# jdubkim/Self-play-on-Multi-Snakes-Environment

Measured on AMD Instinct MI355X. Metric: env-steps/sec (agent·step) at 4 096×19×19×3-snake, 1/2/4/8 GPU + CPU ref, higher is better.
Workload: dtype u8

## Files before the change

### include/msnake.h

```cpp
#ifndef MSNAKE_H
#define MSNAKE_H

#include <stddef.h>
#include <stdint.h>

#ifdef __cplusplus
extern "C" {
#endif

#define MSNAKE_ABI_VERSION 3

#define MSNAKE_RULES_SNAKE_ENV 0
#define MSNAKE_RULES_NEW_WORLD 1
#define MSNAKE_RULES_ADVERSARIAL 2

#define MSNAKE_MAX_SNAKES 4
#define MSNAKE_MAX_FRUITS 32
#define MSNAKE_MAX_DIM 62

#define MSNAKE_OK 0
#define MSNAKE_E_ARG (-1)
#define MSNAKE_E_HIP (-2)
#define MSNAKE_E_HANDLE (-3)
#define MSNAKE_E_ALIGN (-4)
// ... 81 lines not shown
int msnake_state_blob_info(const void* buf, size_t bytes, msnake_blob_info* out);

int msnake_render(msnake_handle h, uint8_t* obs_dev, void* stream);

#define MSNAKE_POLICY_NONE 0
#define MSNAKE_POLICY_SAFE_GREEDY 1
#define MSNAKE_POLICY_HAMILTONIAN 2
int msnake_scripted_actions(msnake_handle h, int32_t policy, uint32_t snake_mask, int32_t* actions_dev,
                            int32_t action_stride, uint8_t* safe_dev, void* stream);

int msnake_copy_envs(msnake_handle dst, msnake_handle src, const int32_t* src_index_dev, void* stream);

int msnake_get_stats(msnake_handle h, msnake_stats* out, int32_t reset);

const char* msnake_kernel_name(msnake_handle h);
int64_t msnake_algorithmic_bytes_per_env_step(msnake_handle h);

#ifdef __cplusplus
}
#endif
#endif
```

### self-play-on-multi-snakes-environment_amd/_capi.py

```python
import ctypes
import os

_HERE = os.path.dirname(os.path.abspath(__file__))
LIB_PATH = os.environ.get("MSNAKE_LIB") or os.path.join(_HERE, "libmsnake.so")

RULES = {"snake_env": 0, "new_world": 1, "adversarial": 2}
RULE_NAMES = {v: k for k, v in RULES.items()}

SYMBOLS = [
    "msnake_abi_version", "msnake_last_error", "msnake_create", "msnake_destroy", "msnake_obs_shape",
    "msnake_reset", "msnake_reset_envs", "msnake_step", "msnake_step_tape", "msnake_rollout_tape", "msnake_get_state", "msnake_set_state",
    "msnake_get_state_all", "msnake_set_state_all", "msnake_state_blob_info",
    "msnake_render", "msnake_get_stats", "msnake_kernel_name", "msnake_algorithmic_bytes_per_env_step",
    "msnake_scripted_actions", "msnake_copy_envs",
]


class MsnakeConfig(ctypes.Structure):
    _fields_ = [("struct_size", ctypes.c_uint32), ("device", ctypes.c_int32), ("num_envs", ctypes.c_int32),
                ("dim", ctypes.c_int32), ("n_snakes", ctypes.c_int32), ("n_fruits", ctypes.c_int32),
                ("rules", ctypes.c_int32), ("max_steps", ctypes.c_int32), ("auto_reset", ctypes.c_int32),
                ("obs_scale", ctypes.c_int32), ("seed", ctypes.c_uint64), ("env_id_base", ctypes.c_uint64),
                ("envs_per_block", ctypes.c_int32), ("record_policy", ctypes.c_int32),
                ("obs_store_policy", ctypes.c_int32), ("tape_store_policy", ctypes.c_int32)]


ABI_VERSION = 3
CONFIG_SIZE_V2 = 56
RECORD_POLICY = {"auto": 0, "full": 1, "short": 2}
# ... 39 lines not shown
    L.msnake_reset_envs.argtypes = [vp, u8p, u8p, u8p, u8p, vp]
    L.msnake_step.argtypes = [vp, vp, i32, u8p, vp, vp, vp, vp]
    L.msnake_scripted_actions.argtypes = [vp, i32, ctypes.c_uint32, vp, i32, u8p, vp]
    L.msnake_copy_envs.argtypes = [vp, vp, vp, vp]
    L.msnake_step_tape.argtypes = [vp, vp, i32, i32, u8p, ctypes.c_size_t, vp, vp, vp, ctypes.c_size_t, vp]
    L.msnake_rollout_tape.argtypes = L.msnake_step_tape.argtypes
    L.msnake_get_state.argtypes = [vp, i32, vp, i32]
    L.msnake_set_state.argtypes = [vp, i32, vp, i32]
    L.msnake_get_state_all.argtypes = [vp, vp, ctypes.c_size_t]
    L.msnake_get_state_all.restype = ctypes.c_int64
    L.msnake_set_state_all.argtypes = [vp, vp, ctypes.c_size_t]
    L.msnake_state_blob_info.argtypes = [vp, ctypes.c_size_t, ctypes.POINTER(MsnakeBlobInfo)]
    L.msnake_get_stats.argtypes = [vp, ctypes.POINTER(MsnakeStats), i32]
    L.msnake_kernel_name.argtypes = [vp]
    L.msnake_kernel_name.restype = ctypes.c_char_p
    L.msnake_algorithmic_bytes_per_env_step.argtypes = [vp]
    L.msnake_algorithmic_bytes_per_env_step.restype = ctypes.c_int64
    for name in ("msnake_create", "msnake_destroy", "msnake_obs_shape", "msnake_reset", "msnake_reset_envs", "msnake_render",
                 "msnake_step", "msnake_step_tape", "msnake_rollout_tape", "msnake_get_state", "msnake_set_state", "msnake_set_state_all",
                 "msnake_state_blob_info", "msnake_get_stats", "msnake_scripted_actions", "msnake_copy_envs"):
        getattr(L, name).restype = ctypes.c_int
    _lib = L
    return L


def check(rc, what="msnake call"):
    if rc < 0:
        msg = load().msnake_last_error().decode("utf-8", "replace")
        raise RuntimeError(f"{what} failed ({rc}): {msg}")
    return rc
```

### self-play-on-multi-snakes-environment_amd/csrc/msnake_capi.hip

```cpp
#include <hip/hip_runtime.h>

#include <cstdarg>
#include <cstdio>
#include <cstdlib>
#include <cstring>
#include <vector>

#include "msnake_internal.h"

namespace {

thread_local char g_err[512] = "";

int fail(int code, const char* fmt, ...) {
    va_list ap;
    va_start(ap, fmt);
    vsnprintf(g_err, sizeof(g_err), fmt, ap);
    va_end(ap);
    return code;
}

#define HIP_TRY(expr)                                                                                   \
    do {                                                                                                \
        hipError_t _e = (expr);                                                                         \
// ... 55 lines not shown
        case 2: return "snake count differs from the handle's";
        case 3: return "fruit count differs from the handle's (or exceeds the fruit-list capacity)";
        case 4: return "a cell lies outside [-1, dim], or a body piece behind the head outside the grid";
        case 5: return "a body length is outside [0, capacity]";
        default: return "malformed state";
    }
}

}

extern "C" {

int msnake_abi_version(void) { return MSNAKE_ABI_VERSION; }
const char* msnake_last_error(void) { return g_err; }

int msnake_create(const msnake_config* cfg_in, msnake_handle* out) {
    if (!cfg_in || !out) return fail(MSNAKE_E_ARG, "msnake_create: NULL argument");
    *out = nullptr;
    if (cfg_in->struct_size != sizeof(msnake_config) && cfg_in->struct_size != MSNAKE_CONFIG_SIZE_V2)
        return fail(MSNAKE_E_ARG, "msnake_config.struct_size %u is neither %zu (ABI 3) nor %u (ABI 2)", cfg_in->struct_size,
                    sizeof(msnake_config), MSNAKE_CONFIG_SIZE_V2);
    msnake_config cfg_full;
    memset(&cfg_full, 0, sizeof(cfg_full));
    memcpy(&cfg_full, cfg_in, cfg_in->struct_size);
    cfg_full.struct_size = (uint32_t)sizeof(msnake_config);
    const msnake_config* cfg = &cfg_full;
    if (cfg->num_envs < 1) return fail(MSNAKE_E_ARG, "num_envs must be >= 1 (got %d)", cfg->num_envs);
    if (cfg->dim < 2 || cfg->dim > MSNAKE_MAX_DIM)
        return fail(MSNAKE_E_ARG, "dim must be in [2, %d] (got %d)", MSNAKE_MAX_DIM, cfg->dim);
    if (cfg->rules != MSNAKE_RULES_SNAKE_ENV && cfg->rules != MSNAKE_RULES_NEW_WORLD &&
        cfg->rules != MSNAKE_RULES_ADVERSARIAL)
        return fail(MSNAKE_E_ARG, "rules %d is not one of MSNAKE_RULES_*", cfg->rules);
    if (cfg->rules == MSNAKE_RULES_NEW_WORLD) {
        if (cfg->n_snakes < 1 || cfg->n_snakes > MSNAKE_MAX_SNAKES)
            return fail(MSNAKE_E_ARG, "new_world: n_snakes must be in [1, %d]", MSNAKE_MAX_SNAKES);
        if (cfg->n_fruits < 0 || cfg->n_fruits > MSNAKE_MAX_FRUITS)
            return fail(MSNAKE_E_ARG, "new_world: n_fruits must be in [0, %d]", MSNAKE_MAX_FRUITS);
    } else {
        if (cfg->n_snakes < 1 || cfg->n_snakes > 3)
            return fail(MSNAKE_E_ARG, "snake_env: n_snakes must be in [1, 3] (got %d)", cfg->n_snakes);
        if (cfg->n_fruits != cfg->n_snakes)
// ... 1 lines not shown
    }
    if (cfg->max_steps < 1 || cfg->max_steps > 60000)
        return fail(MSNAKE_E_ARG, "max_steps must be in [1, 60000]");
    if ((uint64_t)cfg->num_envs * (uint64_t)(MSNAKE_HDR_WORDS * 4 + MSNAKE_MAX_SNAKES * 128) >= (1ull << 32))
        return fail(MSNAKE_E_ARG, "num_envs %d: records and body rings of one handle must stay below 4 GB (the kernel "
                                  "addresses them with 32-bit offsets); use several handles", cfg->num_envs);
    if (cfg->obs_scale != 1 && cfg->obs_scale != 4 && cfg->obs_scale != 7)
        return fail(MSNAKE_E_ARG, "obs_scale must be 1, 4 (21->84) or 7 (12->84), got %d", cfg->obs_scale);
    if (cfg->envs_per_block < 0 || cfg->envs_per_block > MSNAKE_MAX_ENVS_PER_BLOCK)
        return fail(MSNAKE_E_ARG, "envs_per_block must be 0 (auto) or in [1, %d], got %d", MSNAKE_MAX_ENVS_PER_BLOCK, cfg->envs_per_block);
    if (cfg->record_policy < 0 || cfg->record_policy > MSNAKE_RECORD_SHORT)
        return fail(MSNAKE_E_ARG, "record_policy must be MSNAKE_AUTO, MSNAKE_RECORD_FULL or MSNAKE_RECORD_SHORT, got %d", cfg->record_policy);
    if (cfg->obs_store_policy < 0 || cfg->obs_store_policy > MSNAKE_STORE_STREAM || cfg->tape_store_policy < 0 ||
        cfg->tape_store_policy > MSNAKE_STORE_STREAM)
        return fail(MSNAKE_E_ARG, "obs_store_policy / tape_store_policy must be MSNAKE_AUTO, MSNAKE_STORE_PLAIN or MSNAKE_STORE_STREAM");

    int ndev = 0;
    if (hipGetDeviceCount(&ndev) != hipSuccess || ndev < 1)
        return fail(MSNAKE_E_NOGPU, "no HIP device available (this library has no CPU path)");
    if (cfg->device < 0 || cfg->device >= ndev)
        return fail(MSNAKE_E_ARG, "device %d out of range (have %d)", cfg->device, ndev);
    DeviceGuard guard(cfg->device);

    msnake_env* h = static_cast<msnake_env*>(calloc(1, sizeof(msnake_env)));
    if (!h) return fail(MSNAKE_E_ARG, "out of host memory");
    h->cfg = *cfg;
    msnake::StepParams& p = h->p;
    const int dim = cfg->dim, W = dim + 2, n2 = dim * dim;
    p.nenv = cfg->num_envs;
    p.dim = dim;
    p.n_snakes = cfg->n_snakes;
    p.n_fruits = cfg->n_fruits;
    p.views = cfg->rules == MSNAKE_RULES_NEW_WORLD ? cfg->n_snakes : 3;
    p.C = 3 * p.views;
    p.S = W * W * p.C;
    p.obs_scale = cfg->obs_scale;
    p.rest.max_steps = cfg->max_steps;
    p.auto_reset = cfg->auto_reset ? 1 : 0;
    int need = n2 + 2;
    if (cfg->rules == MSNAKE_RULES_NEW_WORLD && cfg->max_steps + 2 > need) need = cfg->max_steps + 2;
    p.rest.cap = (need + 63) / 64 * 64;
    const int K = cfg->obs_scale;
    if (K > 1 && (W * K * p.C) % 4 != 0) {
        free(h);
        return fail(MSNAKE_E_ARG, "obs_scale %d: output rows must be whole dwords", K);
    }
    p.img_bytes = (p.S * K + (K == 1 ? 15 : 0) + 1023) / 1024 * 1024;
    p.rest.seed_lo = (uint32_t)cfg->seed;
    p.rest.seed_hi = (uint32_t)(cfg->seed >> 32);
    p.rest.env_id_base = cfg->env_id_base;
    p.lds_per_wave = p.img_bytes + (n2 + 15) / 16 * 16;
    h->epb = p.nenv <= 8192 ? MSNAKE_MAX_ENVS_PER_BLOCK : 4;
    while (h->epb > 1 && (size_t)h->epb * p.lds_per_wave > 64 * 1024) h->epb >>= 1;
    if ((size_t)p.lds_per_wave > 64 * 1024 - 16 || p.S > 0xFFFF) {
        free(h);
        return fail(MSNAKE_E_ARG, "observation image of %d bytes does not fit in LDS", p.S);
    }

    const size_t hdr_bytes = (size_t)p.nenv * MSNAKE_HDR_WORDS * 4;
    const size_t body0_bytes = (size_t)p.nenv * p.n_snakes * 64 * 2;
    const int tmpl_copies = K == 1 ? MSNAKE_TMPL_COPIES : 1;
    const size_t tmpl_bytes = (size_t)p.img_bytes * tmpl_copies;
    const size_t ring_bytes = (size_t)p.nenv * p.n_snakes * p.rest.cap * 2;
    const bool adv = cfg->rules == MSNAKE_RULES_ADVERSARIAL;
    p.fcap = (p.n_snakes + p.n_snakes * (n2 + 2) + 63) / 64 * 64;
    const size_t fl0_bytes = adv ? (size_t)p.nenv * 64 * 2 : 0;
    const size_t flist_bytes = adv ? (size_t)p.nenv * p.fcap * 2 : 0;
    const size_t state_bytes = hdr_bytes + body0_bytes + tmpl_bytes + ring_bytes + fl0_bytes + flist_bytes;
    hipError_t e;
    if ((e = hipMalloc(&h->d_state, state_bytes)) != hipSuccess || (e = hipMalloc(&h->d_stats, 64)) != hipSuccess ||
        (e = hipMemset(h->d_state, 0, state_bytes)) != hipSuccess || (e = hipMemset(h->d_stats, 0, 64)) != hipSuccess) {
        (void)hipFree(h->d_state); (void)hipFree(h->d_stats);
// ... 8 lines not shown
    p.fl0 = reinterpret_cast<uint16_t*>(p.state + hdr_bytes + body0_bytes + tmpl_bytes + ring_bytes);
    p.flist = reinterpret_cast<uint16_t*>(p.state + hdr_bytes + body0_bytes + tmpl_bytes + ring_bytes + fl0_bytes);
    p.stats = static_cast<unsigned long long*>(h->d_stats);
    std::vector<uint8_t> tmpl(tmpl_bytes, 0);
    for (int copy = 0; copy < tmpl_copies; ++copy)
        for (int r = 0; r < W; ++r)
            for (int c = 0; c < W; ++c)
                if (r == 0 || r == W - 1 || c == 0 || c == W - 1)
                    memset(&tmpl[(size_t)copy * p.img_bytes + copy + ((size_t)r * W + c) * p.C * K], 255, (size_t)p.C * K);
    if ((e = hipMemcpy(const_cast<uint8_t*>(p.tmpl), tmpl.data(), tmpl_bytes, hipMemcpyHostToDevice)) != hipSuccess) {
        (void)hipFree(h->d_state); (void)hipFree(h->d_stats);
        free(h);
        return fail(MSNAKE_E_HIP, "uploading the background image failed: %s", hipGetErrorString(e));
    }
    if (cfg->envs_per_block > 0 && cfg->envs_per_block < h->epb) h->epb = cfg->envs_per_block;
    p.short_rec = (cfg->rules != MSNAKE_RULES_NEW_WORLD && p.nenv > 8192) ? 1 : 0;
    if (cfg->record_policy != MSNAKE_AUTO)
        p.short_rec = (cfg->rules != MSNAKE_RULES_NEW_WORLD && cfg->record_policy == MSNAKE_RECORD_SHORT) ? 1 : 0;
    {
        const double obs_mib = (double)p.nenv * p.S * p.obs_scale * p.obs_scale / (1024.0 * 1024.0);
        p.rest.stream_obs = (p.obs_scale == 1 ? (obs_mib <= 32.0 || obs_mib >= 192.0) : obs_mib >= 400.0) ? 1u : 0u;
    }
    if (cfg->obs_store_policy != MSNAKE_AUTO) p.rest.stream_obs = cfg->obs_store_policy == MSNAKE_STORE_STREAM ? 1u : 0u;
#ifdef MSNAKE_DBG_STAGES
    if (const char* dbg = getenv("MSNAKE_DBG_STAGE")) p.rest.dbg_stage = (uint32_t)atoi(dbg);
    if (const char* dbg = getenv("MSNAKE_DBG_BUF")) p.rest.dbg_buf = reinterpret_cast<unsigned long long*>(strtoull(dbg, nullptr, 0));
#endif
#if defined(MSNAKE_DBG_STAGES) || defined(MSNAKE_SPAN_LIGHT)
    if (const char* dbg = getenv("MSNAKE_DBG_SPAN")) {
        h->dbg_span = reinterpret_cast<unsigned long long*>(strtoull(dbg, nullptr, 0));
        const char* sl = getenv("MSNAKE_DBG_SPAN_SLOTS");
        h->dbg_span_slots = sl ? (uint32_t)atoi(sl) : 1u;
        if (h->dbg_span_slots < 1) h->dbg_span_slots = 1;
    }
#endif
    msnake::step_kernel_name(cfg->rules, cfg->n_snakes, cfg->obs_scale, h->kname, sizeof(h->kname));
    h->magic = kMagic;
    *out = h;
    return MSNAKE_OK;
}

int msnake_destroy(msnake_handle h) {
    if (int rc = check(h)) return rc;
    DeviceGuard guard(h->cfg.device);
    (void)hipDeviceSynchronize();
    (void)hipFree(h->d_state); (void)hipFree(h->d_stats);
    if (h->d_scratch) (void)hipFree(h->d_scratch);
    h->magic = 0;
    free(h);
    return MSNAKE_OK;
}
// ... 309 lines not shown
    memset(out, 0, sizeof(*out));
    out->episodes = (int64_t)raw[0];
    out->ep_len_sum = (int64_t)raw[1];
    out->ep_return_sum = (int64_t)raw[2];
    out->env_steps = h->env_steps;
    out->errors = (int64_t)raw[4];
    if (reset) h->env_steps = 0;
    return MSNAKE_OK;
}

const char* msnake_kernel_name(msnake_handle h) {
    if (check(h)) return "";
    return h->kname;
}

int64_t msnake_algorithmic_bytes_per_env_step(msnake_handle h) {
    if (check(h)) return -1;
    const msnake::StepParams& p = h->p;
    return (int64_t)p.S * p.obs_scale * p.obs_scale + (int64_t)p.dim * p.dim + 4 * p.n_snakes + 5 + 16 * p.n_snakes + 16;
}

}
```

### self-play-on-multi-snakes-environment_amd/csrc/msnake_internal.h

```cpp
#ifndef MSNAKE_INTERNAL_H
#define MSNAKE_INTERNAL_H

#include <hip/hip_runtime.h>
#include <stdint.h>

#include "../../include/msnake.h"

#define MSNAKE_BLOCK_THREADS 512
#define MSNAKE_MAX_ENVS_PER_BLOCK 8

#define MSNAKE_HDR_WORDS 64
#define MSNAKE_HDR_SHORT_WORDS 32
#define SN_A(s) (0 + (s))
#define SN_B(s) (4 + (s))
#define SN_C(s) (8 + (s))
#define SN_C_HP0_SHIFT 24
#define HDR_T 12
#define HDR_CTR_LO 13
#define HDR_CTR_HI 14
#define HDR_FLAGS 15
#define HDR_FLAG_FINISHED 0x100u
#define HDR_EP_RETURN 16
#define HDR_EP_LEN 17
#define HDR_SPARE 18
// ... 38 lines not shown
#define PK2_SHORT_REC 1u
#define PK2_STREAM_OBS 2u
#define PK2_STREAM_TAPE 4u
#define PK2_TAPE_ALIGNED 8u
#define PK2_EPB_SHIFT 8
#define PK2_DIVM_SHIFT 16

struct StepParams {
    int32_t nenv, dim, n_snakes, n_fruits, views, C, S, auto_reset;
    int32_t lds_per_wave;
    int32_t img_bytes;
    int32_t action_stride;
    int32_t obs_scale;
    int32_t short_rec;
    int32_t stream_tape;
    uint8_t* state;
    uint32_t* hdr;
    uint16_t* body0;
    const uint8_t* tmpl;
    uint16_t* ring;
    uint16_t* fl0;
    uint16_t* flist;
    int32_t fcap;
    unsigned long long* stats;
    const int32_t* actions;
    uint8_t* obs;
    StepRest rest;
};

hipError_t launch_stats(uint32_t* hdr, int nenv, unsigned long long* stats, int clear, hipStream_t stream);
hipError_t launch_step(const StepParams& p, int rules, int mode, int envs_per_block, hipStream_t stream);
hipError_t launch_state_sizes(const StepParams& p, int rules, int env0, int count, uint32_t* need_words, hipStream_t stream);
hipError_t launch_state_pack(const StepParams& p, int rules, int env0, int count, const uint64_t* offsets, int32_t* words,
                             hipStream_t stream);
hipError_t launch_state_unpack(const StepParams& p, int rules, int env0, int count, const uint64_t* offsets,
                               const int32_t* words, uint32_t* status, hipStream_t stream);
hipError_t launch_scripted(const StepParams& p, int rules, int policy, uint32_t snake_mask, int32_t* actions, int32_t action_stride,
                           uint8_t* safe, hipStream_t stream);
hipError_t launch_copy_envs(const StepParams& dst, const StepParams& src, int rules, const int32_t* src_index, hipStream_t stream);
void step_kernel_name(int rules, int n_snakes, int obs_scale, char* out, size_t n);

}

#endif
```

### self-play-on-multi-snakes-environment_amd/csrc/msnake_kernels.hip

```cpp
#include <hip/hip_runtime.h>
#include <stdint.h>
#include <stdio.h>
#include <stdlib.h>

#include <type_traits>

#include "msnake_internal.h"

namespace msnake {

__device__ __forceinline__ uint64_t ballot(bool p) { return __builtin_amdgcn_ballot_w64(p); }
__device__ __forceinline__ uint32_t rdlane(uint32_t v, int l) {
    return (uint32_t)__builtin_amdgcn_readlane((int)v, l);
}
__device__ __forceinline__ uint32_t uni(uint32_t v) { return (uint32_t)__builtin_amdgcn_readfirstlane((int)v); }
__device__ __forceinline__ void wave_sync() {
    __builtin_amdgcn_fence(__ATOMIC_RELEASE, "wavefront");
    __builtin_amdgcn_wave_barrier();
    __builtin_amdgcn_fence(__ATOMIC_ACQUIRE, "wavefront");
}
__device__ __forceinline__ uint32_t mbcnt(uint64_t m) {
    return __builtin_amdgcn_mbcnt_hi((uint32_t)(m >> 32), __builtin_amdgcn_mbcnt_lo((uint32_t)m, 0u));
}
template <int N>
// ... 117 lines not shown
        *reinterpret_cast<u16_unaligned*>(p + 4) = head ? H4 : B4;
    } else if constexpr (C == 9) {
        constexpr uint64_t H = pix_word<J, VIEWS, 8>(true, 0), B = pix_word<J, VIEWS, 8>(false, 0);
        constexpr uint8_t H8 = pix_byte<J, VIEWS>(true, 8), B8 = pix_byte<J, VIEWS>(false, 8);
        *reinterpret_cast<u64_unaligned*>(p) = head ? H : B;
        p[8] = head ? H8 : B8;
    } else {
        static_assert(C == 12, "views");
        constexpr uint64_t H = pix_word<J, VIEWS, 8>(true, 0), B = pix_word<J, VIEWS, 8>(false, 0);
        constexpr uint32_t H8 = (uint32_t)pix_word<J, VIEWS, 4>(true, 8), B8 = (uint32_t)pix_word<J, VIEWS, 4>(false, 8);
        *reinterpret_cast<u64_unaligned*>(p) = head ? H : B;
        *reinterpret_cast<u32_unaligned*>(p + 8) = head ? H8 : B8;
    }
}

template <int RULES, int NS, int MODE, int K>
__global__ __launch_bounds__(MSNAKE_BLOCK_THREADS) void msnake_step_kernel(
    uint8_t* __restrict__ state, uint8_t* __restrict__ obs, const int32_t* __restrict__ actions,
    float* __restrict__ rew_out, uint8_t* __restrict__ done_out, const int32_t nenv, const uint32_t pk0,
    const uint32_t pk1, const uint32_t pk2, const StepRest p) {
    constexpr int VIEWS = RULES == MSNAKE_RULES_NEW_WORLD ? NS : 3;
    constexpr int C = 3 * VIEWS;
    extern __shared__ __attribute__((aligned(16))) uint8_t smem[];
    int lane = (int)(threadIdx.x & 63u);
    const int wave = (int)uni(threadIdx.x >> 6);
    const uint32_t epb = (pk2 >> PK2_EPB_SHIFT) & 0xFFu;
    uint32_t b = blockIdx.x;
    b = (b & ~63u) | ((b & 7u) << 3) | ((b >> 3) & 7u);
    const int e = (int)(b * epb) + wave;
    if (e >= nenv) return;
    if ((MODE == 1 || MODE == 2) && p.env_mask && uni(p.env_mask[e]) == 0u) {
        if (MODE == 1 && p.truncated && lane == 0) p.truncated[e] = 0;
        return;
    }

    uint32_t pk0v = pk0, pk1v = pk1, pk2v = pk2;
    int dim, nf, action_stride, S, cap, W, n2, img_bytes, occ_bytes;
    bool auto_reset, short_rec;
    uint32_t max_steps;
    uint8_t *img, *bg;
    constexpr int FR0 = RULES == MSNAKE_RULES_NEW_WORLD ? HDR_FRUIT0_N : HDR_FRUIT0_S;
    constexpr bool LDSBG = MODE == 3 && K == 1;
    constexpr int TMPL_COPIES = K == 1 ? MSNAKE_TMPL_COPIES : 1;
#ifdef MSNAKE_NO_ALIGN
    constexpr bool CAN_ALIGN = false;
#else
    constexpr bool CAN_ALIGN = K == 1;
#endif
    const bool align_now = CAN_ALIGN && (MODE != 3 || (pk2 & PK2_TAPE_ALIGNED));
    auto unpack = [&]() {
        dim = (int)(pk0v & 63u); nf = (int)((pk0v >> 6) & 63u); action_stride = (int)((pk0v >> 12) & 7u);
        auto_reset = (pk0v >> 15) & 1u;
        max_steps = pk0v >> 16;
        S = (int)(pk1v & 0xFFFFu); cap = (int)(pk1v >> 16);
        short_rec = RULES != MSNAKE_RULES_NEW_WORLD && (pk2v & PK2_SHORT_REC);
        W = dim + 2; n2 = dim * dim;
    };
    auto lds_layout = [&]() {
        img_bytes = (S * K + (K == 1 ? 15 : 0) + 1023) & ~1023;
        occ_bytes = (n2 + 15) & ~15;
        img = smem + (size_t)wave * (size_t)(img_bytes + occ_bytes + (LDSBG ? img_bytes : 0));
        bg = img + img_bytes + occ_bytes;
    };
    unpack();
#ifdef MSNAKE_DBG_STAGES
// ... 17 lines not shown
#ifdef MSNAKE_SPAN_LIGHT
    unsigned long long span_t0 = 0;
#define SPAN(k) do { if ((k) == 0) span_t0 = __builtin_amdgcn_s_memrealtime(); \
                     if ((k) == 5 && p.dbg_span && lane == 0) { p.dbg_span[(size_t)e * 8] = span_t0; p.dbg_span[(size_t)e * 8 + 5] = __builtin_amdgcn_s_memrealtime(); } } while (0)
#else
#define SPAN(k) if (p.dbg_span && lane == 0) p.dbg_span[(size_t)e * 8 + (k)] = __builtin_amdgcn_s_memrealtime()
#endif
#define SPAN_FLAG(v) dbgf |= (v)
    uint32_t dbgf = 0;
#else
#define SPAN(k)
#define SPAN_FLAG(v)
#endif
    constexpr bool FENCED = RULES == MSNAKE_RULES_ADVERSARIAL || NS == 4 || MODE == 3;
#define LANE_FENCE() do { if (FENCED) asm volatile("" : "+v"(lane)); } while (0)
#define CONFIG_FENCE() do { if (FENCED && MODE != 3) { asm volatile("" : "+s"(pk0v), "+s"(pk1v), "+s"(pk2v)); unpack(); lds_layout(); } } while (0)

    STAMP(0);
    SPAN(0);
    uint32_t* hdr_g = reinterpret_cast<uint32_t*>(state + (uint32_t)e * (uint32_t)(MSNAKE_HDR_WORDS * 4));
    uint16_t* body0_g = reinterpret_cast<uint16_t*>(state + ((uint32_t)nenv * (uint32_t)(MSNAKE_HDR_WORDS * 4) +
                                                             (uint32_t)e * (uint32_t)(NS * 128)));
    auto tmpl_of = [&]() -> const uint8_t* {
        uint32_t n = (uint32_t)nenv;
        if (MODE == 3) asm volatile("" : "+s"(n));
        return state + n * (uint32_t)(MSNAKE_HDR_WORDS * 4 + NS * 128);
    };
    auto ring_of = [&](int s) -> uint16_t* {
        uint32_t ee = (uint32_t)e;
        asm volatile("" : "+s"(ee));
        return reinterpret_cast<uint16_t*>(const_cast<uint8_t*>(tmpl_of()) + img_bytes * TMPL_COPIES) + ((size_t)ee * NS + (size_t)s) * (size_t)cap;
// ... 182 lines not shown
        int x = 0;
        if (nfree > 0) {
            const uint32_t k = rnd((uint32_t)nfree);
#ifdef MSNAKE_DBG_STAGES
            if (dbg & 0x2000) x = (int)k; else {
#endif
            const int L = __builtin_ffsll((long long)ballot(freescan > k)) - 1;
            const uint64_t m = ((uint64_t)rdlane((uint32_t)(freemask >> 32), L) << 32) | rdlane((uint32_t)freemask, L);
            const uint32_t kk = k - (rdlane(freescan, L) - (uint32_t)__builtin_popcountll(m));
            const uint64_t sel = ballot(((m >> lane) & 1ull) && mbcnt(m) == kk);
            x = L * 64 + (__builtin_ffsll((long long)sel) - 1);
#ifdef MSNAKE_DBG_STAGES
            }
#endif
        }
        uint32_t p2 = pk2v;
        asm volatile("" : "+s"(p2));
        const uint32_t sh = 14u + 32u - (uint32_t)__builtin_clz((uint32_t)dim);
        const uint32_t q = ((uint32_t)x * (p2 >> PK2_DIVM_SHIFT)) >> sh;
        const uint32_t r = (uint32_t)x - q * (uint32_t)dim;
        return ((r + 1u) << 8) | (q + 1u);
    };
    auto safe_cell = [&]() -> uint32_t {
        if (RULES == MSNAKE_RULES_ADVERSARIAL && nfree > 0) ensure_draws(1);
        return pick_cell(randint);
    };

    auto do_reset = [&]() {
        if (RULES == MSNAKE_RULES_NEW_WORLD) {
#pragma unroll
            for (int s = 0; s < NS; ++s) HV_SET_U(SN_A(s), 0u);
        }
        if (RULES != MSNAKE_RULES_NEW_WORLD) {
            const uint32_t ctr_lo = rdlane(hv, HDR_CTR_LO), ctr_hi = rdlane(hv, HDR_CTR_HI);
// ... 60 lines not shown
        do_reset();
        HV_SET_C(HDR_EP_RETURN, 0u);
        HV_SET_C(HDR_EP_LEN, 0u);
    }

    DBG_EXIT(1)
    const int n_steps = MODE == 3 ? p.n_steps : 1;
    float* rew_t = rew_out;
    uint8_t* done_t = done_out;
    msnake_info* info_t = p.info;
    uint8_t* obs_t = obs;
    uint32_t abatch = 0;
#pragma nounroll
    for (int step_i = 0; step_i < n_steps; ++step_i) {
    if (MODE == 3) {
        asm volatile("" : "+v"(lane), "+s"(pk0v), "+s"(pk1v), "+s"(pk2v));
        unpack();
        lds_layout();
        __builtin_amdgcn_s_setprio(0);
    }
    if (MODE == 3) {
        if (step_i > 0) {
            rew_t += p.scalar_step_stride; done_t += p.scalar_step_stride;
            if (info_t) info_t += p.scalar_step_stride;
            if (obs_t) obs_t += p.obs_step_stride;
        }
        if ((step_i & 15) == 0) {
            const int t = step_i + (lane >> 2);
            abatch = 0;
            if ((lane & 3) < NS && t < n_steps)
                abatch = (uint32_t)actions[((size_t)t * (size_t)nenv + (size_t)e) * action_stride + (lane & 3)];
// ... 3 lines not shown
        uint32_t ee = (uint32_t)e;
        if (FENCED) asm volatile("" : "+s"(ee));
        return (align_now && obs_t) ? (((uint32_t)(uintptr_t)obs_t + ee * (uint32_t)S) & 15u) : 0u;
    };
#ifdef MSNAKE_DBG_STAGES
    if (obs_t && (!LDSBG || step_i == 0) && !(dbg & 0x100)) {
#else
    if (obs_t && (!LDSBG || step_i == 0)) {
#endif
        const uint4* tsrc = reinterpret_cast<const uint4*>(tmpl_of() + (CAN_ALIGN ? obs_shift_of() * (uint32_t)img_bytes : 0u)) + lane;
        uint8_t* dst = LDSBG ? bg : img;
        const int nk = img_bytes >> 10;
#define MSNAKE_GP(k) ((const __attribute__((address_space(1))) void*)(tsrc + (k) * 64))
#define MSNAKE_LP(k) ((__attribute__((address_space(3))) void*)(dst + (k) * 1024))
        const uint32_t lds0 = (uint32_t)(uintptr_t)MSNAKE_LP(0);
        asm volatile("s_mov_b32 m0, %1\n\ts_nop 0\n\t"
                     "global_load_lds_dwordx4 %0, off\n\t"
                     "s_cmp_lt_u32 %2, 2\n\ts_cbranch_scc1 1f\n\t"
                     "global_load_lds_dwordx4 %0, off offset:1024\n\t"
                     "s_cmp_lt_u32 %2, 3\n\ts_cbranch_scc1 1f\n\t"
                     "global_load_lds_dwordx4 %0, off offset:2048\n\t"
                     "s_cmp_lt_u32 %2, 4\n\ts_cbranch_scc1 1f\n\t"
                     "global_load_lds_dwordx4 %0, off offset:3072\n"
                     "1:"
                     :: "v"(tsrc), "s"(uni(lds0)), "s"(uni((uint32_t)nk)) : "m0", "scc", "memory");
        if (nk > 4)
            for (int k = 4; k < nk; ++k) __builtin_amdgcn_global_load_lds(MSNAKE_GP(k), MSNAKE_LP(k), 16, 0, 0);
#undef MSNAKE_GP
#undef MSNAKE_LP
    }
// ... 554 lines not shown
            const int lead = (int)(((uint32_t)(uintptr_t)g_al >> 4) & 7u);
            const int end = (int)obs_shift + DBG_NO_OBS_STORES(S);
            const int kmin = (int)((obs_shift + 15u) >> 4);
            const uint32_t nk = (uint32_t)((end >> 4) - kmin);
            const int k0 = lane - lead;
            const uint32_t rel = (uint32_t)(k0 - kmin);
            const uint8_t* lsrc = img + 16 * k0;
            uint8_t* gdst = g_al + 16 * k0;
            auto chunks = [&](auto NT) {
#pragma unroll
                for (int i = 0; i < 4; ++i) {
                    if (rel + 64u * i < nk DBG_FEWER_STORES(i)) {
                        const u32x4 v = *reinterpret_cast<const u32x4*>(lsrc + 1024 * i);
                        if constexpr (decltype(NT)::value) __builtin_nontemporal_store(v, reinterpret_cast<u32x4*>(gdst + 1024 * i));
                        else *reinterpret_cast<u32x4*>(gdst + 1024 * i) = v;
                    }
                }
                if (nk + (uint32_t)(kmin + lead) > 256u)
                    for (uint32_t r = rel + 256u; r < nk; r += 64u) {
                        const u32x4 v = *reinterpret_cast<const u32x4*>(lsrc + 16 * (r - rel));
                        if constexpr (decltype(NT)::value) __builtin_nontemporal_store(v, reinterpret_cast<u32x4*>(gdst + 16 * (size_t)(r - rel)));
                        else *reinterpret_cast<u32x4*>(gdst + 16 * (size_t)(r - rel)) = v;
                    }
            };
            if (pk2 & (MODE == 3 ? PK2_STREAM_TAPE : PK2_STREAM_OBS)) chunks(std::true_type{});
            else chunks(std::false_type{});
            const bool head = lane < 16;
            const int byte = head ? lane : (end & ~15) + (lane - 16);
            const uint32_t first = head ? obs_shift : 16u;
            const uint32_t count = head ? ((16u - obs_shift) & 15u) : ((uint32_t)end & 15u);
            if ((uint32_t)lane - first < count) g_al[byte] = img[byte];
        } else if (K == 1) {
            uint8_t* obs_env = obs_t + (size_t)e * S;
// ... 314 lines not shown
}

hipError_t launch_state_unpack(const StepParams& p, int rules, int env0, int count, const uint64_t* offsets,
                               const int32_t* words, uint32_t* status, hipStream_t stream) {
    hipLaunchKernelGGL(msnake_state_unpack_kernel, dim3((unsigned)((count + 3) / 4)), dim3(256), 0, stream,
                       state_view(p, rules), env0, count, offsets, words, status);
    return hipGetLastError();
}

static uint32_t div_magic(uint32_t dim) {
    uint32_t bits = 0;
    while ((dim >> bits) != 0) ++bits;
    return (uint32_t)((1ull << (14u + bits)) / dim) + 1u;
}

template <int RULES, int NS, int K>
static hipError_t launch_k(const StepParams& p, int mode, int epb, hipStream_t stream) {
    const uint32_t pk0 = (uint32_t)p.dim | ((uint32_t)p.n_fruits << 6) | ((uint32_t)p.action_stride << 12) |
                         ((uint32_t)(p.auto_reset ? 1 : 0) << 15) | ((uint32_t)p.rest.max_steps << 16);
    const uint32_t pk1 = (uint32_t)p.S | ((uint32_t)p.rest.cap << 16);

    size_t lds_wave = (size_t)p.lds_per_wave;
    if (mode == 3 && K == 1) {
        lds_wave += (size_t)p.img_bytes;
        while (epb > 1 && lds_wave * (size_t)epb > 64 * 1024) epb >>= 1;
        if (lds_wave > 64 * 1024) return hipErrorInvalidValue;
    }
    const size_t lds = lds_wave * (size_t)epb;
    bool nt_obs = p.rest.stream_obs != 0;
    if (K > 1) {
        const size_t OB = (size_t)p.S * K * K;
        nt_obs = nt_obs && mode != 3 && p.obs && OB % 16 == 0 && ((uintptr_t)p.obs & 15) == 0 && OB < (1u << 24);
    }
    const uint32_t pk2 = (p.short_rec ? PK2_SHORT_REC : 0u) | (nt_obs ? PK2_STREAM_OBS : 0u) |
                         (p.stream_tape && K == 1 ? PK2_STREAM_TAPE : 0u) |
                         (mode == 3 && K == 1 && p.rest.obs_step_stride % 16 == 0 ? PK2_TAPE_ALIGNED : 0u) | ((uint32_t)epb << PK2_EPB_SHIFT) |
                         (div_magic((uint32_t)p.dim) << PK2_DIVM_SHIFT);
    const dim3 grid((unsigned)((((p.nenv + epb - 1) / epb) + 63) & ~63));
    const dim3 block(64u * (unsigned)epb);
#define MSNAKE_LAUNCH(M)                                                                                       \
    hipLaunchKernelGGL((msnake_step_kernel<RULES, NS, M, K>), grid, block, lds, stream, p.state, p.obs, p.actions, \
                       p.rest.rew, p.rest.done, p.nenv, pk0, pk1, pk2, p.rest)
    switch (mode) {
        case 0: MSNAKE_LAUNCH(0); break;
        case 1: MSNAKE_LAUNCH(1); break;
        case 3: MSNAKE_LAUNCH(3); break;
        default: MSNAKE_LAUNCH(2); break;
    }
#undef MSNAKE_LAUNCH
    return hipGetLastError();
}

template <int RULES, int NS>
static hipError_t launch_ns(const StepParams& p, int mode, int epb, hipStream_t stream) {
    switch (p.obs_scale) {
        case 1: return launch_k<RULES, NS, 1>(p, mode, epb, stream);
        case 4: return launch_k<RULES, NS, 4>(p, mode, epb, stream);
        case 7: return launch_k<RULES, NS, 7>(p, mode, epb, stream);
        default: return hipErrorInvalidValue;
    }
}

template <int RULES>
static hipError_t launch_rules(const StepParams& p, int mode, int epb, hipStream_t stream) {
// ... 6 lines not shown
            return hipErrorInvalidValue;
        default: return hipErrorInvalidValue;
    }
}

hipError_t launch_step(const StepParams& p, int rules, int mode, int epb, hipStream_t stream) {
    if (epb < 1 || epb > MSNAKE_MAX_ENVS_PER_BLOCK) return hipErrorInvalidValue;
    switch (rules) {
        case MSNAKE_RULES_SNAKE_ENV: return launch_rules<MSNAKE_RULES_SNAKE_ENV>(p, mode, epb, stream);
        case MSNAKE_RULES_NEW_WORLD: return launch_rules<MSNAKE_RULES_NEW_WORLD>(p, mode, epb, stream);
        case MSNAKE_RULES_ADVERSARIAL: return launch_rules<MSNAKE_RULES_ADVERSARIAL>(p, mode, epb, stream);
        default: return hipErrorInvalidValue;
    }
}

void step_kernel_name(int rules, int n_snakes, int obs_scale, char* out, size_t n) {
    snprintf(out, n, "msnake_step_kernel<%d, %d, 0, %d>", rules, n_snakes, obs_scale);
}

}

#include "msnake_scripted.inc"
#include "msnake_copy.inc"
```

### self-play-on-multi-snakes-environment_amd/vec_env.py

```python
import ctypes
import time

import numpy as np

from . import _capi
from .spaces import Box, Discrete

GYM_IDS = {
    "snake-multiple-test-v0": dict(rules="snake_env", dim=19),
    "snake-new-multiple-v0": dict(rules="new_world", dim=10),
    "snake-adversarial-v0": dict(rules="adversarial", dim=10),
}


def normalize_actions(actions, num_envs, n_snakes):
    a = np.asarray(actions)
    if a.ndim == 1:
        a = a[:, None]
    if a.ndim != 2 or a.shape[0] != num_envs:
        raise ValueError(f"expected {num_envs} action rows, got array of shape {a.shape}")
    if a.shape[1] < n_snakes:
        raise ValueError(f"each action row needs >= {n_snakes} entries, got {a.shape[1]}")
    return np.ascontiguousarray(a, dtype=np.int32)

# ... 94 lines not shown
            raise ValueError("terminal_obs=True needs auto_reset=True (it replaces the in-kernel auto reset)")
        if n_fruits is None:
            n_fruits = n_snakes
        self._ctor = dict(dim=dim, n_snakes=n_snakes, n_fruits=n_fruits, rules=rules, seed=seed, env_id_base=env_id_base,
                          device=self.device, max_steps=max_steps, auto_reset=auto_reset, obs_scale=obs_scale,
                          declared_channels=declared_channels, host_views=host_views, envs_per_block=envs_per_block,
                          record_policy=record_policy, obs_store_policy=obs_store_policy,
                          tape_store_policy=tape_store_policy, terminal_obs=terminal_obs)
        self.cfg = _capi.MsnakeConfig(ctypes.sizeof(_capi.MsnakeConfig), self.device.index or 0, int(num_envs),
                                      int(dim), int(n_snakes), int(n_fruits), rules_id, int(max_steps),
                                      int(bool(auto_reset) and not self.terminal_obs), int(obs_scale), int(seed),
                                      int(env_id_base),
                                      int(envs_per_block), _capi.RECORD_POLICY[record_policy],
                                      _capi.STORE_POLICY[obs_store_policy], _capi.STORE_POLICY[tape_store_policy])
        self._h = ctypes.c_void_p()
        _capi.check(self._L.msnake_create(ctypes.byref(self.cfg), ctypes.byref(self._h)), "msnake_create")
        H, W, C = ctypes.c_int32(), ctypes.c_int32(), ctypes.c_int32()
        _capi.check(self._L.msnake_obs_shape(self._h, ctypes.byref(H), ctypes.byref(W), ctypes.byref(C)))
        self.num_envs = int(num_envs)
        self.n_snakes = int(n_snakes)
        self.rules = _capi.RULE_NAMES[rules_id]
        self.obs_shape = (H.value, W.value, C.value)
        self.observation_space = Box(0, 255, (H.value, W.value, declared_channels or C.value), np.uint8)
        self.action_space = Discrete(5)
        with torch.cuda.device(self.device):
            self._obs = torch.empty((self.num_envs,) + self.obs_shape, dtype=torch.uint8, device=self.device)
            self._rew = torch.zeros(self.num_envs, dtype=torch.float32, device=self.device)
            self._done = torch.zeros(self.num_envs, dtype=torch.uint8, device=self.device)
            self._info = torch.zeros((self.num_envs, 4), dtype=torch.int32, device=self.device)
            self.final_obs = self.truncated = None
# ... 305 lines not shown
```

Baseline: 746.3 million.

## Add compile-time-shape specialized step kernels for common snake_env configurations

Adds a DIM template parameter to the step kernel so that snake_env at dim 19 (2 or 3 snakes) and dim 10 (1 snake) get constant-folded shapes, divide magic, LDS layouts and unrolled LDS-load sequences. Runtime config unpacking and the config fences are skipped in that path. Host code picks the specialized kernel when the config matches and offers an env-var switch back to the generic kernels. The cost is more kernel instantiations and a larger binary, plus the chance of a subtle mismatch between the specialized path and the runtime-derived shapes.

```diff
diff --git a/include/msnake.h b/include/msnake.h
--- a/include/msnake.h
+++ b/include/msnake.h
@@ -119,6 +119,8 @@
 int msnake_get_stats(msnake_handle h, msnake_stats* out, int32_t reset);
 
 const char* msnake_kernel_name(msnake_handle h);
+int msnake_kernel_name_for_config(const msnake_config* cfg, char* out, size_t n);
+int msnake_set_generic_kernels(int32_t on);
 int64_t msnake_algorithmic_bytes_per_env_step(msnake_handle h);
 
 #ifdef __cplusplus
diff --git a/self-play-on-multi-snakes-environment_amd/_capi.py b/self-play-on-multi-snakes-environment_amd/_capi.py
--- a/self-play-on-multi-snakes-environment_amd/_capi.py
+++ b/self-play-on-multi-snakes-environment_amd/_capi.py
@@ -12,7 +12,8 @@
     "msnake_reset", "msnake_reset_envs", "msnake_step", "msnake_step_tape", "msnake_rollout_tape", "msnake_get_state", "msnake_set_state",
     "msnake_get_state_all", "msnake_set_state_all", "msnake_state_blob_info",
     "msnake_render", "msnake_get_stats", "msnake_kernel_name", "msnake_algorithmic_bytes_per_env_step",
-    "msnake_scripted_actions", "msnake_copy_envs",
+    "msnake_scripted_actions", "msnake_copy_envs", "msnake_kernel_name_for_config",
+    "msnake_set_generic_kernels",
 ]
 
 
@@ -82,6 +83,10 @@
     L.msnake_get_stats.argtypes = [vp, ctypes.POINTER(MsnakeStats), i32]
     L.msnake_kernel_name.argtypes = [vp]
     L.msnake_kernel_name.restype = ctypes.c_char_p
+    L.msnake_kernel_name_for_config.argtypes = [ctypes.POINTER(MsnakeConfig), ctypes.c_char_p, ctypes.c_size_t]
+    L.msnake_kernel_name_for_config.restype = ctypes.c_int
+    L.msnake_set_generic_kernels.argtypes = [i32]
+    L.msnake_set_generic_kernels.restype = ctypes.c_int
     L.msnake_algorithmic_bytes_per_env_step.argtypes = [vp]
     L.msnake_algorithmic_bytes_per_env_step.restype = ctypes.c_int64
     for name in ("msnake_create", "msnake_destroy", "msnake_obs_shape", "msnake_reset", "msnake_reset_envs", "msnake_render",
@@ -92,6 +97,17 @@
     return L
 
 
+def apply_kernel_switch():
+    load().msnake_set_generic_kernels(int(os.environ.get("MSNAKE_GENERIC_KERNELS", "") not in ("", "0")))
+
+
+def kernel_name_for_config(cfg):
+    apply_kernel_switch()
+    buf = ctypes.create_string_buffer(64)
+    check(load().msnake_kernel_name_for_config(ctypes.byref(cfg), buf, len(buf)), "msnake_kernel_name_for_config")
+    return buf.value.decode()
+
+
 def check(rc, what="msnake call"):
     if rc < 0:
         msg = load().msnake_last_error().decode("utf-8", "replace")
diff --git a/self-play-on-multi-snakes-environment_amd/csrc/msnake_capi.hip b/self-play-on-multi-snakes-environment_amd/csrc/msnake_capi.hip
--- a/self-play-on-multi-snakes-environment_amd/csrc/msnake_capi.hip
+++ b/self-play-on-multi-snakes-environment_amd/csrc/msnake_capi.hip
@@ -1,5 +1,6 @@
 #include <hip/hip_runtime.h>
 
+#include <atomic>
 #include <cstdarg>
 #include <cstdio>
 #include <cstdlib>
@@ -93,17 +94,16 @@
 int msnake_abi_version(void) { return MSNAKE_ABI_VERSION; }
 const char* msnake_last_error(void) { return g_err; }
 
-int msnake_create(const msnake_config* cfg_in, msnake_handle* out) {
-    if (!cfg_in || !out) return fail(MSNAKE_E_ARG, "msnake_create: NULL argument");
-    *out = nullptr;
+namespace {
+
+int validate_config(const msnake_config* cfg_in, msnake_config* cfg_full) {
     if (cfg_in->struct_size != sizeof(msnake_config) && cfg_in->struct_size != MSNAKE_CONFIG_SIZE_V2)
         return fail(MSNAKE_E_ARG, "msnake_config.struct_size %u is neither %zu (ABI 3) nor %u (ABI 2)", cfg_in->struct_size,
                     sizeof(msnake_config), MSNAKE_CONFIG_SIZE_V2);
-    msnake_config cfg_full;
-    memset(&cfg_full, 0, sizeof(cfg_full));
-    memcpy(&cfg_full, cfg_in, cfg_in->struct_size);
-    cfg_full.struct_size = (uint32_t)sizeof(msnake_config);
-    const msnake_config* cfg = &cfg_full;
+    memset(cfg_full, 0, sizeof(*cfg_full));
+    memcpy(cfg_full, cfg_in, cfg_in->struct_size);
+    cfg_full->struct_size = (uint32_t)sizeof(msnake_config);
+    const msnake_config* cfg = cfg_full;
     if (cfg->num_envs < 1) return fail(MSNAKE_E_ARG, "num_envs must be >= 1 (got %d)", cfg->num_envs);
     if (cfg->dim < 2 || cfg->dim > MSNAKE_MAX_DIM)
         return fail(MSNAKE_E_ARG, "dim must be in [2, %d] (got %d)", MSNAKE_MAX_DIM, cfg->dim);
@@ -135,18 +135,10 @@
     if (cfg->obs_store_policy < 0 || cfg->obs_store_policy > MSNAKE_STORE_STREAM || cfg->tape_store_policy < 0 ||
         cfg->tape_store_policy > MSNAKE_STORE_STREAM)
         return fail(MSNAKE_E_ARG, "obs_store_policy / tape_store_policy must be MSNAKE_AUTO, MSNAKE_STORE_PLAIN or MSNAKE_STORE_STREAM");
-
-    int ndev = 0;
-    if (hipGetDeviceCount(&ndev) != hipSuccess || ndev < 1)
-        return fail(MSNAKE_E_NOGPU, "no HIP device available (this library has no CPU path)");
-    if (cfg->device < 0 || cfg->device >= ndev)
-        return fail(MSNAKE_E_ARG, "device %d out of range (have %d)", cfg->device, ndev);
-    DeviceGuard guard(cfg->device);
-
-    msnake_env* h = static_cast<msnake_env*>(calloc(1, sizeof(msnake_env)));
-    if (!h) return fail(MSNAKE_E_ARG, "out of host memory");
-    h->cfg = *cfg;
-    msnake::StepParams& p = h->p;
+    return MSNAKE_OK;
+}
+
+int derive_shape(const msnake_config* cfg, msnake::StepParams& p) {
     const int dim = cfg->dim, W = dim + 2, n2 = dim * dim;
     p.nenv = cfg->num_envs;
     p.dim = dim;
@@ -162,21 +154,55 @@
     if (cfg->rules == MSNAKE_RULES_NEW_WORLD && cfg->max_steps + 2 > need) need = cfg->max_steps + 2;
     p.rest.cap = (need + 63) / 64 * 64;
     const int K = cfg->obs_scale;
-    if (K > 1 && (W * K * p.C) % 4 != 0) {
+    if (K > 1 && (W * K * p.C) % 4 != 0) return fail(MSNAKE_E_ARG, "obs_scale %d: output rows must be whole dwords", K);
+    p.img_bytes = (p.S * K + (K == 1 ? 15 : 0) + 1023) / 1024 * 1024;
+    p.lds_per_wave = p.img_bytes + (n2 + 15) / 16 * 16;
+    if ((size_t)p.lds_per_wave > 64 * 1024 - 16 || p.S > 0xFFFF)
+        return fail(MSNAKE_E_ARG, "observation image of %d bytes does not fit in LDS", p.S);
+    p.short_rec = (cfg->rules != MSNAKE_RULES_NEW_WORLD && p.nenv > 8192) ? 1 : 0;
+    if (cfg->record_policy != MSNAKE_AUTO)
+        p.short_rec = (cfg->rules != MSNAKE_RULES_NEW_WORLD && cfg->record_policy == MSNAKE_RECORD_SHORT) ? 1 : 0;
+    return MSNAKE_OK;
+}
+
+std::atomic<int> g_generic_kernels{0};
+
+int pick_spec_dim(const msnake::StepParams& p, int rules) {
+    if (g_generic_kernels.load(std::memory_order_relaxed)) return 0;
+    return msnake::spec_dim_of(p, rules);
+}
+
+}
+
+int msnake_create(const msnake_config* cfg_in, msnake_handle* out) {
+    if (!cfg_in || !out) return fail(MSNAKE_E_ARG, "msnake_create: NULL argument");
+    *out = nullptr;
+    msnake_config cfg_full;
+    if (int rc = validate_config(cfg_in, &cfg_full)) return rc;
+    const msnake_config* cfg = &cfg_full;
+
+    int ndev = 0;
+    if (hipGetDeviceCount(&ndev) != hipSuccess || ndev < 1)
+        return fail(MSNAKE_E_NOGPU, "no HIP device available (this library has no CPU path)");
+    if (cfg->device < 0 || cfg->device >= ndev)
+        return fail(MSNAKE_E_ARG, "device %d out of range (have %d)", cfg->device, ndev);
+    DeviceGuard guard(cfg->device);
+
+    msnake_env* h = static_cast<msnake_env*>(calloc(1, sizeof(msnake_env)));
+    if (!h) return fail(MSNAKE_E_ARG, "out of host memory");
+    h->cfg = *cfg;
+    msnake::StepParams& p = h->p;
+    if (int rc = derive_shape(cfg, p)) {
         free(h);
-        return fail(MSNAKE_E_ARG, "obs_scale %d: output rows must be whole dwords", K);
-    }
-    p.img_bytes = (p.S * K + (K == 1 ? 15 : 0) + 1023) / 1024 * 1024;
+        return rc;
+    }
+    const int dim = cfg->dim, W = dim + 2, n2 = dim * dim;
+    const int K = cfg->obs_scale;
     p.rest.seed_lo = (uint32_t)cfg->seed;
     p.rest.seed_hi = (uint32_t)(cfg->seed >> 32);
     p.rest.env_id_base = cfg->env_id_base;
-    p.lds_per_wave = p.img_bytes + (n2 + 15) / 16 * 16;
     h->epb = p.nenv <= 8192 ? MSNAKE_MAX_ENVS_PER_BLOCK : 4;
     while (h->epb > 1 && (size_t)h->epb * p.lds_per_wave > 64 * 1024) h->epb >>= 1;
-    if ((size_t)p.lds_per_wave > 64 * 1024 - 16 || p.S > 0xFFFF) {
-        free(h);
-        return fail(MSNAKE_E_ARG, "observation image of %d bytes does not fit in LDS", p.S);
-    }
 
     const size_t hdr_bytes = (size_t)p.nenv * MSNAKE_HDR_WORDS * 4;
     const size_t body0_bytes = (size_t)p.nenv * p.n_snakes * 64 * 2;
@@ -215,9 +241,6 @@
         return fail(MSNAKE_E_HIP, "uploading the background image failed: %s", hipGetErrorString(e));
     }
     if (cfg->envs_per_block > 0 && cfg->envs_per_block < h->epb) h->epb = cfg->envs_per_block;
-    p.short_rec = (cfg->rules != MSNAKE_RULES_NEW_WORLD && p.nenv > 8192) ? 1 : 0;
-    if (cfg->record_policy != MSNAKE_AUTO)
-        p.short_rec = (cfg->rules != MSNAKE_RULES_NEW_WORLD && cfg->record_policy == MSNAKE_RECORD_SHORT) ? 1 : 0;
     {
         const double obs_mib = (double)p.nenv * p.S * p.obs_scale * p.obs_scale / (1024.0 * 1024.0);
         p.rest.stream_obs = (p.obs_scale == 1 ? (obs_mib <= 32.0 || obs_mib >= 192.0) : obs_mib >= 400.0) ? 1u : 0u;
@@ -235,7 +258,8 @@
         if (h->dbg_span_slots < 1) h->dbg_span_slots = 1;
     }
 #endif
-    msnake::step_kernel_name(cfg->rules, cfg->n_snakes, cfg->obs_scale, h->kname, sizeof(h->kname));
+    p.spec_dim = pick_spec_dim(p, cfg->rules);
+    msnake::step_kernel_name(cfg->rules, cfg->n_snakes, cfg->obs_scale, p.spec_dim, h->kname, sizeof(h->kname));
     h->magic = kMagic;
     *out = h;
     return MSNAKE_OK;
@@ -575,6 +599,19 @@
     return h->kname;
 }
 
+int msnake_kernel_name_for_config(const msnake_config* cfg_in, char* out, size_t n) {
+    if (!cfg_in || !out || n == 0) return fail(MSNAKE_E_ARG, "msnake_kernel_name_for_config: NULL argument");
+    msnake_config cfg;
+    if (int rc = validate_config(cfg_in, &cfg)) return rc;
+    msnake::StepParams p;
+    memset(&p, 0, sizeof(p));
+    if (int rc = derive_shape(&cfg, p)) return rc;
+    msnake::step_kernel_name(cfg.rules, cfg.n_snakes, cfg.obs_scale, pick_spec_dim(p, cfg.rules), out, n);
+    return MSNAKE_OK;
+}
+
+int msnake_set_generic_kernels(int32_t on) { return g_generic_kernels.exchange(on ? 1 : 0, std::memory_order_relaxed); }
+
 int64_t msnake_algorithmic_bytes_per_env_step(msnake_handle h) {
     if (check(h)) return -1;
     const msnake::StepParams& p = h->p;
diff --git a/self-play-on-multi-snakes-environment_amd/csrc/msnake_internal.h b/self-play-on-multi-snakes-environment_amd/csrc/msnake_internal.h
--- a/self-play-on-multi-snakes-environment_amd/csrc/msnake_internal.h
+++ b/self-play-on-multi-snakes-environment_amd/csrc/msnake_internal.h
@@ -76,6 +76,7 @@
     int32_t obs_scale;
     int32_t short_rec;
     int32_t stream_tape;
+    int32_t spec_dim;
     uint8_t* state;
     uint32_t* hdr;
     uint16_t* body0;
@@ -100,7 +101,8 @@
 hipError_t launch_scripted(const StepParams& p, int rules, int policy, uint32_t snake_mask, int32_t* actions, int32_t action_stride,
                            uint8_t* safe, hipStream_t stream);
 hipError_t launch_copy_envs(const StepParams& dst, const StepParams& src, int rules, const int32_t* src_index, hipStream_t stream);
-void step_kernel_name(int rules, int n_snakes, int obs_scale, char* out, size_t n);
+int spec_dim_of(const StepParams& p, int rules);
+void step_kernel_name(int rules, int n_snakes, int obs_scale, int spec_dim, char* out, size_t n);
 
 }
 
diff --git a/self-play-on-multi-snakes-environment_amd/csrc/msnake_kernels.hip b/self-play-on-multi-snakes-environment_amd/csrc/msnake_kernels.hip
--- a/self-play-on-multi-snakes-environment_amd/csrc/msnake_kernels.hip
+++ b/self-play-on-multi-snakes-environment_amd/csrc/msnake_kernels.hip
@@ -155,13 +155,16 @@
     }
 }
 
-template <int RULES, int NS, int MODE, int K>
+template <int RULES, int NS, int MODE, int K, int DIM = 0>
 __global__ __launch_bounds__(MSNAKE_BLOCK_THREADS) void msnake_step_kernel(
     uint8_t* __restrict__ state, uint8_t* __restrict__ obs, const int32_t* __restrict__ actions,
     float* __restrict__ rew_out, uint8_t* __restrict__ done_out, const int32_t nenv, const uint32_t pk0,
     const uint32_t pk1, const uint32_t pk2, const StepRest p) {
     constexpr int VIEWS = RULES == MSNAKE_RULES_NEW_WORLD ? NS : 3;
     constexpr int C = 3 * VIEWS;
+    constexpr bool SPEC = DIM > 0;
+    static_assert(!SPEC || (RULES == MSNAKE_RULES_SNAKE_ENV && K == 1 && (MODE == 0 || MODE == 3) && DIM <= MSNAKE_MAX_DIM),
+                  "compile-time shapes: snake_env, native size, step / tape kernels");
     extern __shared__ __attribute__((aligned(16))) uint8_t smem[];
     int lane = (int)(threadIdx.x & 63u);
     const int wave = (int)uni(threadIdx.x >> 6);
@@ -190,6 +193,13 @@
 #endif
     const bool align_now = CAN_ALIGN && (MODE != 3 || (pk2 & PK2_TAPE_ALIGNED));
     auto unpack = [&]() {
+        if constexpr (SPEC) {
+            dim = DIM; nf = NS; action_stride = NS; auto_reset = true; short_rec = false;
+            max_steps = pk0v >> 16;
+            S = (DIM + 2) * (DIM + 2) * C; cap = (DIM * DIM + 2 + 63) / 64 * 64;
+            W = DIM + 2; n2 = DIM * DIM;
+            return;
+        }
         dim = (int)(pk0v & 63u); nf = (int)((pk0v >> 6) & 63u); action_stride = (int)((pk0v >> 12) & 7u);
         auto_reset = (pk0v >> 15) & 1u;
         max_steps = pk0v >> 16;
@@ -237,7 +247,7 @@
 #endif
     constexpr bool FENCED = RULES == MSNAKE_RULES_ADVERSARIAL || NS == 4 || MODE == 3;
 #define LANE_FENCE() do { if (FENCED) asm volatile("" : "+v"(lane)); } while (0)
-#define CONFIG_FENCE() do { if (FENCED && MODE != 3) { asm volatile("" : "+s"(pk0v), "+s"(pk1v), "+s"(pk2v)); unpack(); lds_layout(); } } while (0)
+#define CONFIG_FENCE() do { if (FENCED && MODE != 3 && !SPEC) { asm volatile("" : "+s"(pk0v), "+s"(pk1v), "+s"(pk2v)); unpack(); lds_layout(); } } while (0)
 
     STAMP(0);
     SPAN(0);
@@ -450,10 +460,17 @@
             }
 #endif
         }
-        uint32_t p2 = pk2v;
-        asm volatile("" : "+s"(p2));
-        const uint32_t sh = 14u + 32u - (uint32_t)__builtin_clz((uint32_t)dim);
-        const uint32_t q = ((uint32_t)x * (p2 >> PK2_DIVM_SHIFT)) >> sh;
+        uint32_t q;
+        if constexpr (SPEC) {
+            constexpr uint32_t SH = 14u + 32u - (uint32_t)__builtin_clz((uint32_t)DIM);
+            constexpr uint32_t M = (1u << SH) / (uint32_t)DIM + 1u;
+            q = ((uint32_t)x * M) >> SH;
+        } else {
+            uint32_t p2 = pk2v;
+            asm volatile("" : "+s"(p2));
+            const uint32_t sh = 14u + 32u - (uint32_t)__builtin_clz((uint32_t)dim);
+            q = ((uint32_t)x * (p2 >> PK2_DIVM_SHIFT)) >> sh;
+        }
         const uint32_t r = (uint32_t)x - q * (uint32_t)dim;
         return ((r + 1u) << 8) | (q + 1u);
     };
@@ -544,7 +561,8 @@
 #pragma nounroll
     for (int step_i = 0; step_i < n_steps; ++step_i) {
     if (MODE == 3) {
-        asm volatile("" : "+v"(lane), "+s"(pk0v), "+s"(pk1v), "+s"(pk2v));
+        if (SPEC) asm volatile("" : "+v"(lane), "+s"(pk0v));
+        else asm volatile("" : "+v"(lane), "+s"(pk0v), "+s"(pk1v), "+s"(pk2v));
         unpack();
         lds_layout();
         __builtin_amdgcn_s_setprio(0);
@@ -578,6 +596,20 @@
 #define MSNAKE_GP(k) ((const __attribute__((address_space(1))) void*)(tsrc + (k) * 64))
 #define MSNAKE_LP(k) ((__attribute__((address_space(3))) void*)(dst + (k) * 1024))
         const uint32_t lds0 = (uint32_t)(uintptr_t)MSNAKE_LP(0);
+        constexpr int NK_SPEC = SPEC ? ((DIM + 2) * (DIM + 2) * C + 15 + 1023) >> 10 : 0;
+        if constexpr (NK_SPEC == 4)
+            asm volatile("s_mov_b32 m0, %1\n\ts_nop 0\n\t"
+                         "global_load_lds_dwordx4 %0, off\n\t"
+                         "global_load_lds_dwordx4 %0, off offset:1024\n\t"
+                         "global_load_lds_dwordx4 %0, off offset:2048\n\t"
+                         "global_load_lds_dwordx4 %0, off offset:3072"
+                         :: "v"(tsrc), "s"(uni(lds0)) : "m0", "memory");
+        else if constexpr (NK_SPEC == 2)
+            asm volatile("s_mov_b32 m0, %1\n\ts_nop 0\n\t"
+                         "global_load_lds_dwordx4 %0, off\n\t"
+                         "global_load_lds_dwordx4 %0, off offset:1024"
+                         :: "v"(tsrc), "s"(uni(lds0)) : "m0", "memory");
+        else
         asm volatile("s_mov_b32 m0, %1\n\ts_nop 0\n\t"
                      "global_load_lds_dwordx4 %0, off\n\t"
                      "s_cmp_lt_u32 %2, 2\n\ts_cbranch_scc1 1f\n\t"
@@ -1162,9 +1194,13 @@
                         const u32x4 v = *reinterpret_cast<const u32x4*>(lsrc + 1024 * i);
                         if constexpr (decltype(NT)::value) __builtin_nontemporal_store(v, reinterpret_cast<u32x4*>(gdst + 1024 * i));
                         else *reinterpret_cast<u32x4*>(gdst + 1024 * i) = v;
+                        if constexpr (SPEC) {
+                            if constexpr (decltype(NT)::value) asm volatile("; streaming copy-out" ::: "memory");
+                            else asm volatile("; plain copy-out" ::: "memory");
+                        }
                     }
                 }
-                if (nk + (uint32_t)(kmin + lead) > 256u)
+                if ((!SPEC || ((S + 15) >> 4) + 7 > 256) && nk + (uint32_t)(kmin + lead) > 256u)
                     for (uint32_t r = rel + 256u; r < nk; r += 64u) {
                         const u32x4 v = *reinterpret_cast<const u32x4*>(lsrc + 16 * (r - rel));
                         if constexpr (decltype(NT)::value) __builtin_nontemporal_store(v, reinterpret_cast<u32x4*>(gdst + 16 * (size_t)(r - rel)));
@@ -1509,6 +1545,22 @@
     return (uint32_t)((1ull << (14u + bits)) / dim) + 1u;
 }
 
+static constexpr bool has_spec(int rules, int ns, int k, int dim) {
+    return rules == MSNAKE_RULES_SNAKE_ENV && k == 1 && ((dim == 19 && (ns == 2 || ns == 3)) || (dim == 10 && ns == 1));
+}
+int spec_dim_of(const StepParams& p, int rules) {
+    if (!has_spec(rules, p.n_snakes, p.obs_scale, p.dim)) return 0;
+    const int W = p.dim + 2, n2 = p.dim * p.dim, S = W * W * 9;
+    if (p.n_fruits != p.n_snakes || !p.auto_reset || p.short_rec || p.views != 3 || p.C != 9) return 0;
+    if (p.S != S || p.rest.cap != (n2 + 2 + 63) / 64 * 64 || p.img_bytes != ((S + 15 + 1023) & ~1023) ||
+        p.lds_per_wave != p.img_bytes + ((n2 + 15) & ~15))
+        return 0;
+    return p.dim;
+}
+static int spec_dim_now(const StepParams& p, int mode) {
+    return (p.spec_dim != 0 && (mode == 0 || mode == 3) && p.action_stride == p.n_snakes) ? p.spec_dim : 0;
+}
+
 template <int RULES, int NS, int K>
 static hipError_t launch_k(const StepParams& p, int mode, int epb, hipStream_t stream) {
     const uint32_t pk0 = (uint32_t)p.dim | ((uint32_t)p.n_fruits << 6) | ((uint32_t)p.action_stride << 12) |
@@ -1533,9 +1585,18 @@
                          (div_magic((uint32_t)p.dim) << PK2_DIVM_SHIFT);
     const dim3 grid((unsigned)((((p.nenv + epb - 1) / epb) + 63) & ~63));
     const dim3 block(64u * (unsigned)epb);
-#define MSNAKE_LAUNCH(M)                                                                                       \
-    hipLaunchKernelGGL((msnake_step_kernel<RULES, NS, M, K>), grid, block, lds, stream, p.state, p.obs, p.actions, \
+#define MSNAKE_LAUNCH_D(M, D)                                                                                     \
+    hipLaunchKernelGGL((msnake_step_kernel<RULES, NS, M, K, D>), grid, block, lds, stream, p.state, p.obs, p.actions, \
                        p.rest.rew, p.rest.done, p.nenv, pk0, pk1, pk2, p.rest)
+#define MSNAKE_LAUNCH(M) MSNAKE_LAUNCH_D(M, 0)
+    constexpr int SPEC_DIM = has_spec(RULES, NS, K, 19) ? 19 : has_spec(RULES, NS, K, 10) ? 10 : 0;
+    if constexpr (SPEC_DIM != 0) {
+        if (spec_dim_now(p, mode) == SPEC_DIM) {
+            if (mode == 0) MSNAKE_LAUNCH_D(0, SPEC_DIM);
+            else MSNAKE_LAUNCH_D(3, SPEC_DIM);
+            return hipGetLastError();
+        }
+    }
     switch (mode) {
         case 0: MSNAKE_LAUNCH(0); break;
         case 1: MSNAKE_LAUNCH(1); break;
@@ -1543,6 +1604,7 @@
         default: MSNAKE_LAUNCH(2); break;
     }
 #undef MSNAKE_LAUNCH
+#undef MSNAKE_LAUNCH_D
     return hipGetLastError();
 }
 
@@ -1579,8 +1641,9 @@
     }
 }
 
-void step_kernel_name(int rules, int n_snakes, int obs_scale, char* out, size_t n) {
-    snprintf(out, n, "msnake_step_kernel<%d, %d, 0, %d>", rules, n_snakes, obs_scale);
+void step_kernel_name(int rules, int n_snakes, int obs_scale, int spec_dim, char* out, size_t n) {
+    if (spec_dim != 0) snprintf(out, n, "msnake_step_kernel<%d, %d, 0, %d, %d>", rules, n_snakes, obs_scale, spec_dim);
+    else snprintf(out, n, "msnake_step_kernel<%d, %d, 0, %d>", rules, n_snakes, obs_scale);
 }
 
 }
diff --git a/self-play-on-multi-snakes-environment_amd/vec_env.py b/self-play-on-multi-snakes-environment_amd/vec_env.py
--- a/self-play-on-multi-snakes-environment_amd/vec_env.py
+++ b/self-play-on-multi-snakes-environment_amd/vec_env.py
@@ -132,6 +132,7 @@
                                       int(envs_per_block), _capi.RECORD_POLICY[record_policy],
                                       _capi.STORE_POLICY[obs_store_policy], _capi.STORE_POLICY[tape_store_policy])
         self._h = ctypes.c_void_p()
+        _capi.apply_kernel_switch()
         _capi.check(self._L.msnake_create(ctypes.byref(self.cfg), ctypes.byref(self._h)), "msnake_create")
         H, W, C = ctypes.c_int32(), ctypes.c_int32(), ctypes.c_int32()
         _capi.check(self._L.msnake_obs_shape(self._h, ctypes.byref(H), ctypes.byref(W), ctypes.byref(C)))
```

After: 776.1 million, median of 6. +4.0%, better.
